# PRBonn/LiDiff

Measured on NVIDIA H100. Metric: denoising_steps_per_sec_180k_pts_T50, higher is better.
Workload: dtype fp16x3 split tensor-core MMA, fp32 accumulate (fp32 CUDA cores for the Cin=3 stem), fp64 DPM update

## Files before the change

lidiff_b200/csrc/common.cuh:

```cuda
#pragma once
#include <cuda_runtime.h>
#include <stdint.h>
#include <stdio.h>
#include <string.h>
#include "../../include/lidiff_b200.h"

struct Lb2Handle {
    int      device;
    int      num_sms;
    int64_t  launches;
    int32_t* d_status;
    uint32_t configured;
    char     err[512];
};

enum { LB2_K_TC = 0, LB2_K_SCATTER = 4, LB2_K_NN_TABLE = 8, LB2_K_FPS_CLUSTER = 9, LB2_K_WGRAD = 10 };
template <class K>
static inline cudaError_t lb2_configure_smem(Lb2Handle* h, int bit, K kernel, int bytes) {
    if (h->configured & (1u << bit)) return cudaSuccess;
    cudaError_t e = cudaFuncSetAttribute(kernel, cudaFuncAttributeMaxDynamicSharedMemorySize, bytes);
    if (e == cudaSuccess) h->configured |= 1u << bit;
    return e;
}

static inline int lb2_fail(Lb2Handle* h, int code, const char* fmt, const char* a = "", const char* b = "") {
    if (h) snprintf(h->err, sizeof(h->err), fmt, a, b);
    return code;
}

#define LB2_POST_LAUNCH(h, name)                                                              \
    do {                                                                                      \
        (h)->launches++;                                                                      \
        cudaError_t e__ = cudaGetLastError();                                                 \
        if (e__ != cudaSuccess) return lb2_fail((h), LB2_ERR_CUDA, "%s: %s", name, cudaGetErrorString(e__)); \
    } while (0)

#define LB2_REQUIRE(h, cond, msg)                                                             \
    do { if (!(cond)) return lb2_fail((h), LB2_ERR_ARG, "bad argument: %s", msg); } while (0)

static inline unsigned cdiv(long long a, long long b) { return (unsigned)((a + b - 1) / b); }

size_t rs_sort_scratch_bytes(int n_cap, int nbits);
int rs_sort_keys(Lb2Handle* h, cudaStream_t s, const unsigned* keys, const int* d_n, int n_cap, int nbits, int* order, void* scratch);

#define LB2_AXIS_BITS 18
#define LB2_AXIS_OFF  (1 << (LB2_AXIS_BITS - 1))

__device__ __forceinline__ bool lb2_pack_key(int b, int x, int y, int z, unsigned long long& key) {
    unsigned ux = (unsigned)x + LB2_AXIS_OFF, uy = (unsigned)y + LB2_AXIS_OFF, uz = (unsigned)z + LB2_AXIS_OFF;
    const unsigned lim = 1u << LB2_AXIS_BITS;
    bool ok = ((unsigned)b < 1024u) && ux < lim && uy < lim && uz < lim;
    if (!ok) {
        b = min(max(b, 0), 1023);
        ux = min(ux, lim - 1); uy = min(uy, lim - 1); uz = min(uz, lim - 1);
        if (x < -LB2_AXIS_OFF) ux = 0;
        if (y < -LB2_AXIS_OFF) uy = 0;
        if (z < -LB2_AXIS_OFF) uz = 0;
    }
    key = ((unsigned long long)b << (3 * LB2_AXIS_BITS)) | ((unsigned long long)ux << (2 * LB2_AXIS_BITS))
        | ((unsigned long long)uy << LB2_AXIS_BITS) | (unsigned long long)uz;
    return ok;
}

__device__ __forceinline__ unsigned lb2_hash(unsigned long long k) {
    k ^= k >> 33; k *= 0xff51afd7ed558ccdULL; k ^= k >> 33; k *= 0xc4ceb9fe1a85ec53ULL; k ^= k >> 33;
    return (unsigned)k;
}

#define LB2_MAP_AXIS_OFF (1 << (LB2_MAP_AXIS_BITS - 1))

template <class T>
__device__ __forceinline__ bool lb2_map_cell_ok(T f) { return f >= -(T)LB2_MAP_AXIS_OFF && f < (T)LB2_MAP_AXIS_OFF; }

__device__ __forceinline__ unsigned long long lb2_map_key_push(unsigned long long key, int cell) {
    return (key << LB2_MAP_AXIS_BITS) | (unsigned long long)(unsigned)(cell + LB2_MAP_AXIS_OFF);
}

__device__ __forceinline__ unsigned lb2_key_insert(unsigned long long* keys, unsigned mask, unsigned long long key) {
    unsigned s = lb2_hash(key) & mask;
    while (true) {
        unsigned long long kk = keys[s];
        if (kk == LB2_KEY_EMPTY) {
            kk = atomicCAS(keys + s, (unsigned long long)LB2_KEY_EMPTY, key);
            if (kk == LB2_KEY_EMPTY) return s;
        }
        if (kk == key) return s;
        s = (s + 1) & mask;
    }
}

__device__ __forceinline__ int lb2_grid_lookup(const unsigned long long* __restrict__ keys,
                                               const int* __restrict__ rows, unsigned mask,
                                               unsigned long long key) {
    unsigned slot = lb2_hash(key) & mask;
    while (true) {
        unsigned long long kk = __ldg(keys + slot);
        if (kk == key) return __ldg(rows + slot);
        if (kk == LB2_KEY_EMPTY) return -1;
        slot = (slot + 1) & mask;
    }
}

__device__ __forceinline__ int floor_to_multiple(int v, int ts) {
    int q = v / ts;
    if ((v % ts != 0) && ((v < 0) != (ts < 0))) --q;
    return q * ts;
}
```

lidiff_b200/csrc/spconv_tc.cu:

```cuda
#include "common.cuh"
#include <algorithm>
#include <stdlib.h>
#include "tc_common.cuh"

namespace tc {

constexpr int THREADS = 384;
constexpr int NUM_PRODUCER = 128;
constexpr int NUM_CONSUMER_WARPS = 8;
constexpr int STEP_BUDGET = 64;
constexpr int MAX_KVOL = 27;
constexpr int MAX_STAGES = 4;
constexpr int EPI_BATCH = 4;

struct Params {
    int c1, c2, cout, kvol;
    const unsigned char* wpacked;
    const float* scale;
    const float* shift;
    int relu;
    const int* nbr;
    long long nbr_stride;
    const int* d_mout;
    int mout_cap;
    const int* row_perm;
    const unsigned* row_mask;
    const int* tile_order;
    int stages, nchunks, group;
    int npass, nsplit;
    lb2_conv_io io[2];
    uint32_t range_mask, prior_mask;
    const float* partial_in;
    float* partial_out;
};

constexpr int PRODUCER_REGS = 88;
constexpr int CONSUMER_REGS = 208;
static_assert(128 * PRODUCER_REGS + 256 * CONSUMER_REGS <= THREADS * 168, "register split exceeds the CTA's allocation");

struct TileInfo {
    int idx[MAX_KVOL * BM];
    int row[BM];
    uint32_t mask[4];
    uint32_t prior[4];
    int item;
    int pad[3];
};
constexpr int NUM_BARS = 3 * MAX_STAGES + 4;

template <int NC>
__global__ void __launch_bounds__(THREADS, 1) k_spconv_tc(const Params p) {
    extern __shared__ unsigned char smem_raw[];
    const int M = p.d_mout ? min(*p.d_mout, p.mout_cap) : p.mout_cap;
    const int warp = threadIdx.x >> 5, lane = threadIdx.x & 31;
    const int ctot = p.c1 + p.c2;
    const int S = p.stages;

    const uint32_t raw = smem_u32(smem_raw);
    const uint32_t base = (raw + 1023u) & ~1023u;
    unsigned char* gen = smem_raw + (base - raw);
    constexpr uint32_t b_tile = (uint32_t)NC * 128u;
    const uint32_t b_full = (uint32_t)p.cout * 128u;
    const uint32_t stage_bytes = 2u * A_TILE + 2u * b_tile;
    TileInfo* info = reinterpret_cast<TileInfo*>(gen + (size_t)S * stage_bytes);
    const uint32_t bar0 = smem_u32(info + 2);
    auto full_a = [&](int s) { return bar0 + 8u * s; };
    auto full_b = [&](int s) { return bar0 + 8u * (MAX_STAGES + s); };
    auto empty = [&](int s) { return bar0 + 8u * (2 * MAX_STAGES + s); };
    auto info_full = [&](int b) { return bar0 + 8u * (3 * MAX_STAGES + b); };
    auto info_empty = [&](int b) { return bar0 + 8u * (3 * MAX_STAGES + 2 + b); };

    if (threadIdx.x == 0) {
        for (int s = 0; s < S; ++s) { mbar_init(full_a(s), NUM_PRODUCER); mbar_init(full_b(s), 1); mbar_init(empty(s), NUM_CONSUMER_WARPS); }
        for (int b = 0; b < 2; ++b) { mbar_init(info_full(b), NUM_PRODUCER); mbar_init(info_empty(b), NUM_CONSUMER_WARPS); }
        asm volatile("fence.mbarrier_init.release.cluster;" ::: "memory");
    }
    __syncthreads();

    if (warpgroup_role() == 0) {
        setmaxnreg_dec<PRODUCER_REGS>();
        const int sub = threadIdx.x & 7;
        const int rbase = threadIdx.x >> 3;
        const int D = max(S - 2, 0);
        int it = 0, arrived = 0;
        auto tile_of = [&](int x) {
            const int slot_i = x / (p.nsplit * p.npass);
            return slot_i * BM >= p.mout_cap ? -1 : p.tile_order ? __ldg(p.tile_order + slot_i) : slot_i;
        };
        auto load_row = [&](int tile) {
            const int slot = tile * BM + threadIdx.x;
            return (tile >= 0 && slot < M) ? (p.row_perm ? __ldg(p.row_perm + slot) : slot) : -1;
        };
        auto load_indices = [&](int& row, int (&v)[MAX_KVOL]) {
            const uint32_t m = row < 0 ? 0u : (p.row_mask ? __ldg(p.row_mask + row) : ~0u);
            const uint32_t want = m & p.range_mask;
#pragma unroll
            for (int k = 0; k < MAX_KVOL; ++k) {
                v[k] = -1;
                if (k < p.kvol && (want >> k) & 1u) v[k] = p.nbr ? __ldg(p.nbr + (long long)k * p.nbr_stride + row) : row;
            }
            if (m & p.prior_mask) row |= 1 << 30;
        };
        int x = blockIdx.x, tile = tile_of(x), row = load_row(tile), v[MAX_KVOL];
        load_indices(row, v);
        for (int j = 0;; ++j) {
            TileInfo& ti = info[j & 1];
            mbar_wait(info_empty(j & 1), ((j >> 1) & 1) ^ 1);
            if (tile < 0 || tile * BM >= M) {
                if (threadIdx.x == 0) ti.item = -1;
                mbar_arrive(info_full(j & 1));
                break;
            }
            {
                ti.row[threadIdx.x] = row < 0 ? row : row & ~(1 << 30);
                uint32_t have = 0;
#pragma unroll
                for (int k = 0; k < MAX_KVOL; ++k) {
                    if (k < p.kvol) {
                        ti.idx[k * BM + threadIdx.x] = v[k];
                        if (v[k] >= 0) have |= 1u << k;
                    }
                }
                const uint32_t wmask = __reduce_or_sync(0xffffffffu, have);
                const uint32_t wprior = __ballot_sync(0xffffffffu, row >= 0 && (row >> 30));
                if (lane == 0) { ti.mask[warp] = wmask; ti.prior[warp] = wprior; }
                if (threadIdx.x == 0) ti.item = x;
            }
            mbar_arrive(info_full(j & 1));
            mbar_wait(info_full(j & 1), (j >> 1) & 1);
            const uint32_t kmask = ti.mask[0] | ti.mask[1] | ti.mask[2] | ti.mask[3];
            const int x_next = x + gridDim.x;
            const int tile_next = tile_of(x_next);
            const int n0 = (x % p.nsplit) * NC;
            const lb2_conv_io io = p.io[(x / p.nsplit) % p.npass];
            const bool use_h = (io.in1_h != nullptr) && (p.c2 == 0 || io.in2_h != nullptr);
            for (uint32_t km = kmask; km; km &= km - 1) {
                const int k = __ffs(km) - 1;
                const int* idxk = ti.idx + k * BM;
                int src[8];
#pragma unroll
                for (int r = 0; r < 8; ++r) src[r] = idxk[rbase + 16 * r];
                for (int c = 0; c < p.nchunks; ++c) {
                    const int s = it % S;
                    mbar_wait(empty(s), ((it / S) & 1) ^ 1);
                    unsigned char* a_hi = gen + (size_t)s * stage_bytes;
                    const uint32_t a_hi_u = base + (uint32_t)s * stage_bytes;
                    if (threadIdx.x == 0) {
                        const uint32_t dst = a_hi_u + 2u * A_TILE;
                        const unsigned char* wsrc = p.wpacked + PACK_HEADER + ((size_t)k * p.nchunks + c) * (2u * b_full) + (size_t)n0 * 128u;
                        mbar_expect_tx(full_b(s), 2u * b_tile);
                        bulk_g2s(dst, wsrc, b_tile, full_b(s));
                        bulk_g2s(dst + b_tile, wsrc + b_full, b_tile, full_b(s));
                    }
                    const int ch = c * KC + sub * 8;
                    if (ch < ctot) {
                        const bool first = ch < p.c1;
                        const int cw = first ? p.c1 : p.c2;
                        const int co = first ? ch : ch - p.c1;
                        if (use_h) produce_a_split(reinterpret_cast<const __half*>(first ? io.in1_h : io.in2_h), cw, co, src, a_hi_u, a_hi_u + A_TILE, rbase, sub);
                        else produce_a_f32(first ? io.in1 : io.in2, cw, co, src, a_hi, a_hi + A_TILE, rbase, sub);
                    }
                    cp_async_commit();
                    ++it;
                    if (it - arrived > D) {
                        cp_async_wait_dyn(D);
                        fence_proxy_async();
                        mbar_arrive(full_a(arrived % S));
                        ++arrived;
                    }
                }
            }
            const int s = it % S;
            mbar_wait(empty(s), ((it / S) & 1) ^ 1);
            if (threadIdx.x == 0) mbar_arrive(full_b(s));
            ++it;
            x = x_next;
            tile = tile_next;
            row = load_row(tile);
            cp_async_wait<0>();
            fence_proxy_async();
            for (; arrived < it; ++arrived) mbar_arrive(full_a(arrived % S));
            load_indices(row, v);
        }
    } else {
        setmaxnreg_inc<CONSUMER_REGS>();
        const int wg = (warp >> 2) - 1;
        const float out_scale = __ldg(reinterpret_cast<const float*>(p.wpacked) + 1);
        int it = 0;
        for (int j = 0;; ++j) {
            const TileInfo& ti = info[j & 1];
            mbar_wait(info_full(j & 1), (j >> 1) & 1);
            const int x = ti.item;
            if (x < 0) break;
            const int n_off = __popc(ti.mask[0] | ti.mask[1] | ti.mask[2] | ti.mask[3]);
            float acc[NC / 2], tot[NC / 2];
            if (p.partial_in) {
                const int r0 = wg * 64 + (warp & 3) * 16 + (lane >> 2);
                const float* src[2];
#pragma unroll
                for (int hh = 0; hh < 2; ++hh) {
                    const int rr = r0 + 8 * hh;
                    const bool pr = (ti.prior[rr >> 5] >> (rr & 31)) & 1u;
                    src[hh] = pr ? p.partial_in + ((long long)((x / p.nsplit) % p.npass) * p.mout_cap + ti.row[rr]) * p.cout + (x % p.nsplit) * NC
                                 : nullptr;
                }
#pragma unroll
                for (int i = 0; i < NC / 2; i += 2) {
                    const float* q = src[(i >> 1) & 1];
                    const float2 t = q ? __ldcg(reinterpret_cast<const float2*>(q + 8 * (i >> 2) + 2 * (lane & 3))) : make_float2(-0.f, -0.f);
                    tot[i] = t.x;
                    tot[i + 1] = t.y;
                }
            } else {
#pragma unroll
                for (int i = 0; i < NC / 2; ++i) tot[i] = -0.f;
            }
            const int n_it = n_off * p.nchunks;
            int c = 0, in_group = 0, off_idx = 0, prev_s = -1;
            for (int i = 0; i < n_it; ++i, ++it) {
                const int s = it % S;
                const uint32_t par = (it / S) & 1;
                mbar_wait(full_b(s), par);
                mbar_wait(full_a(s), par);
                const uint32_t a_hi = base + (uint32_t)s * stage_bytes + (uint32_t)wg * (A_TILE / 2), a_lo = a_hi + A_TILE;
                const uint32_t b_hi = base + (uint32_t)s * stage_bytes + 2u * A_TILE, b_lo = b_hi + b_tile;
                const int ksteps = min(KC, ctot - c * KC) >> 4;
                reg_fence(acc);
                wg_stage_mma<NC>(acc, a_hi, a_lo, b_hi, b_lo, ksteps, in_group == 0 && c == 0);
                reg_fence(acc);
                wgmma_wait<1>();
                if (prev_s >= 0 && lane == 0) mbar_arrive(empty(prev_s));
                prev_s = s;
                if (++c < p.nchunks) continue;
                c = 0;
                ++off_idx;
                if (++in_group == p.group || off_idx == n_off) {
                    wgmma_wait<0>();
                    reg_fence(acc);
                    if (lane == 0) mbar_arrive(empty(prev_s));
                    prev_s = -1;
#pragma unroll
                    for (int i = 0; i < NC / 2; ++i) tot[i] = __fadd_rn(tot[i], acc[i]);
                    in_group = 0;
                }
            }
            wgmma_wait<0>();
            const int se = it % S;
            mbar_wait(full_b(se), (it / S) & 1);
            mbar_wait(full_a(se), (it / S) & 1);
            ++it;
            float* stage_c = reinterpret_cast<float*>(gen + (size_t)se * stage_bytes);
            {
                const int r0 = wg * 64 + (warp & 3) * 16 + (lane >> 2);
                const float sc = p.partial_out ? 1.f : out_scale;
#pragma unroll
                for (int i = 0; i < NC / 2; i += 2) {
                    const int row = r0 + 8 * ((i >> 1) & 1), col = 8 * (i >> 2) + 2 * (lane & 3);
                    *reinterpret_cast<float2*>(stage_c + row * NC + (((col >> 2) ^ (row & 7)) << 2) + (col & 3)) =
                        make_float2(tot[i] * sc, tot[i + 1] * sc);
                }
            }
            asm volatile("bar.sync 1, 256;" ::: "memory");
            const lb2_conv_io io = p.io[(x / p.nsplit) % p.npass];
            const int n0 = (x % p.nsplit) * NC;
            const int cw = warp - 4;
            constexpr int nv = NC >> 2;
            constexpr int PER_LANE = (BM / NUM_CONSUMER_WARPS) * nv / 32;
            static_assert(PER_LANE % EPI_BATCH == 0, "a lane's elements come in whole batches");
            const bool has_res = io.residual || io.residual_h;
            const bool gated = io.out_gated || io.out_gated_h;
            const float4 zero4 = make_float4(0.f, 0.f, 0.f, 0.f);
            if (p.partial_out) {
                float* dst = p.partial_out + (long long)((x / p.nsplit) % p.npass) * p.mout_cap * p.cout;
                for (int e = lane; e < PER_LANE * 32; e += 32) {
                    const int rr = cw + NUM_CONSUMER_WARPS * (e / nv);
                    const int lcol = (e % nv) * 4;
                    const int orow = ti.row[rr];
                    if (orow >= 0)
                        __stcg(reinterpret_cast<float4*>(dst + (long long)orow * p.cout + n0 + lcol),
                               *reinterpret_cast<const float4*>(stage_c + rr * NC + (((lcol >> 2) ^ (rr & 7)) << 2)));
                }
            }
            for (int e0 = 0; !p.partial_out && e0 < PER_LANE; e0 += EPI_BATCH) {
                int orow[EPI_BATCH], col[EPI_BATCH];
                long long gi[EPI_BATCH];
                float4 a4[EPI_BATCH], pre4[EPI_BATCH], s4[EPI_BATCH], h4[EPI_BATCH], res4[EPI_BATCH], g4[EPI_BATCH];
#pragma unroll
                for (int b = 0; b < EPI_BATCH; ++b) {
                    const int e = lane + 32 * (e0 + b);
                    const int rr = cw + NUM_CONSUMER_WARPS * (e / nv);
                    const int lcol = (e % nv) * 4;
                    col[b] = n0 + lcol;
                    orow[b] = ti.row[rr];
                    const bool live = orow[b] >= 0;
                    const long long ro = (long long)orow[b] * p.cout;
                    a4[b] = *reinterpret_cast<const float4*>(stage_c + rr * NC + (((lcol >> 2) ^ (rr & 7)) << 2));
                    pre4[b] = (live && io.pre_add) ? __ldg(reinterpret_cast<const float4*>(io.pre_add + ro + col[b])) : zero4;
                    s4[b] = p.scale ? __ldg(reinterpret_cast<const float4*>(p.scale + col[b])) : zero4;
                    h4[b] = p.scale ? __ldg(reinterpret_cast<const float4*>(p.shift + col[b])) : zero4;
                    res4[b] = (live && has_res) ? load_residual4(io.residual, io.residual_h, orow[b], p.cout, col[b]) : zero4;
                    gi[b] = (live && gated && io.gate_table && io.gate_idx) ? __ldg(io.gate_idx + orow[b]) : 0;
                }
#pragma unroll
                for (int b = 0; b < EPI_BATCH; ++b)
                    g4[b] = (orow[b] >= 0 && gated && io.gate_table) ? __ldg(reinterpret_cast<const float4*>(io.gate_table + gi[b] * p.cout + col[b])) : zero4;
#pragma unroll
                for (int b = 0; b < EPI_BATCH; ++b) {
                    if (orow[b] < 0) continue;
                    const long long ro = (long long)orow[b] * p.cout;
                    float y[4] = {a4[b].x, a4[b].y, a4[b].z, a4[b].w};
                    if (io.pre_add) {
                        y[0] += pre4[b].x; y[1] += pre4[b].y; y[2] += pre4[b].z; y[3] += pre4[b].w;
                    }
                    if (p.scale) {
                        y[0] = fmaf(y[0], s4[b].x, h4[b].x); y[1] = fmaf(y[1], s4[b].y, h4[b].y);
                        y[2] = fmaf(y[2], s4[b].z, h4[b].z); y[3] = fmaf(y[3], s4[b].w, h4[b].w);
                    }
                    if (has_res) {
                        y[0] += res4[b].x; y[1] += res4[b].y; y[2] += res4[b].z; y[3] += res4[b].w;
                    }
                    if (p.relu) {
#pragma unroll
                        for (int q = 0; q < 4; ++q) y[q] = fmaxf(y[q], 0.f);
                    }
                    if (io.out) *reinterpret_cast<float4*>(io.out + ro + col[b]) = make_float4(y[0], y[1], y[2], y[3]);
                    if (io.out_h) store_split4(io.out_h, orow[b], p.cout, col[b], y);
                    if (gated) {
                        if (io.gate_table) {
                            y[0] *= g4[b].x; y[1] *= g4[b].y; y[2] *= g4[b].z; y[3] *= g4[b].w;
                        }
                        if (io.out_gated) *reinterpret_cast<float4*>(io.out_gated + ro + col[b]) = make_float4(y[0], y[1], y[2], y[3]);
                        if (io.out_gated_h) store_split4(io.out_gated_h, orow[b], p.cout, col[b], y);
                    }
                }
            }
            fence_proxy_async();
            __syncwarp();
            if (lane == 0) {
                mbar_arrive(empty(se));
                mbar_arrive(info_empty(j & 1));
            }
        }
    }
}

__global__ void k_pack_weights(const float* __restrict__ w, int kvol, int cin, int cout, int nchunks, unsigned char* __restrict__ out) {
    const long long total = (long long)kvol * nchunks * cout * KC;
    long long t = (long long)blockIdx.x * blockDim.x + threadIdx.x;
    const float scale = weight_scale(*reinterpret_cast<const unsigned*>(out));
    if (t == 0) reinterpret_cast<float*>(out)[1] = 1.0f / scale;
    if (t >= total) return;
    const int kk = (int)(t % KC);
    const int n = (int)((t / KC) % cout);
    const int c = (int)((t / ((long long)KC * cout)) % nchunks);
    const int k = (int)(t / ((long long)KC * cout * nchunks));
    const int ch = c * KC + kk;
    const float v = ch < cin ? w[((long long)k * cin + ch) * cout + n] * scale : 0.f;
    const __half hi = __float2half_rn(v);
    const __half lo = __float2half_rn(v - __half2float(hi));
    const size_t tile = (size_t)cout * 128;
    unsigned char* blob = out + PACK_HEADER + ((size_t)k * nchunks + c) * 2 * tile;
    const uint32_t off = sw128(n, kk >> 3) + (uint32_t)(kk & 7) * 2u;
    *reinterpret_cast<__half*>(blob + off) = hi;
    *reinterpret_cast<__half*>(blob + tile + off) = lo;
}

static bool shape_ok(int c1, int c2, int cout, int kvol) {
    const int ctot = c1 + c2;
    if (kvol < 1 || kvol > MAX_KVOL) return false;
    if (ctot % 16 != 0 || ctot < 16) return false;
    if (c2 > 0 && (c1 % 8 != 0 || c2 % 8 != 0)) return false;
    if (cout % 32 != 0 || cout < 32 || cout > 256) return false;
    if (cout > 128 && cout != 256) return false;
    return true;
}

static size_t smem_bytes(int nc, int stages) {
    return 1024 + (size_t)stages * (2 * A_TILE + 2 * (size_t)nc * 128) + 2 * sizeof(TileInfo) + NUM_BARS * sizeof(uint64_t);
}

template <int NC>
static int launch(Lb2Handle* h, cudaStream_t s, const Params& p, int stages) {
    const size_t smem = smem_bytes(NC, stages);
    cudaError_t e = lb2_configure_smem(h, LB2_K_TC + (NC / 32 - 1), k_spconv_tc<NC>, (int)(227 * 1024));
    if (e != cudaSuccess) return lb2_fail(h, LB2_ERR_CUDA, "k_spconv_tc smem attribute: %s", cudaGetErrorString(e));
    const unsigned grid = (unsigned)std::min<long long>(h->num_sms, (long long)cdiv(p.mout_cap, BM) * p.npass * p.nsplit);
    k_spconv_tc<NC><<<grid, THREADS, smem, s>>>(p);
    LB2_POST_LAUNCH(h, "k_spconv_tc");
    return LB2_OK;
}

}

bool lb2_spconv_tc_supported(const lb2_conv_desc* d) { return tc::shape_ok(d->c1, d->c2, d->cout, d->kvol); }

extern "C" size_t lb2_packed_weight_bytes(int32_t kvol, int32_t cin, int32_t cout) {
    if (!tc::shape_ok(cin, 0, cout, kvol)) return 0;
    const int nchunks = (cin + tc::KC - 1) / tc::KC;
    return tc::PACK_HEADER + (size_t)kvol * nchunks * 2 * (size_t)cout * 128;
}

extern "C" int lb2_pack_weights(void* handle, void* stream, const float* weight, int32_t kvol, int32_t cin, int32_t cout, void* packed) {
    Lb2Handle* h = (Lb2Handle*)handle;
    LB2_REQUIRE(h, h && weight && packed, "pack_weights null");
    if (!tc::shape_ok(cin, 0, cout, kvol)) return lb2_fail(h, LB2_ERR_UNSUP, "pack_weights: shape not supported by the tensor-core variant%s", "");
    const int nchunks = (cin + tc::KC - 1) / tc::KC;
    const long long total = (long long)kvol * nchunks * cout * tc::KC;
    const long long nw = (long long)kvol * cin * cout;
    if (cudaMemsetAsync(packed, 0, tc::PACK_HEADER, (cudaStream_t)stream) != cudaSuccess) return lb2_fail(h, LB2_ERR_CUDA, "pack_weights memset%s", "");
    tc::k_weight_absmax<<<(unsigned)std::min<long long>(cdiv(nw, 256), 1024), 256, 0, (cudaStream_t)stream>>>(weight, nw, (unsigned*)packed);
    LB2_POST_LAUNCH(h, "k_weight_absmax");
    tc::k_pack_weights<<<cdiv(total, 256), 256, 0, (cudaStream_t)stream>>>(weight, kvol, cin, cout, nchunks, (unsigned char*)packed);
    LB2_POST_LAUNCH(h, "k_pack_weights");
    return LB2_OK;
}

int lb2_spconv_tc_launch(Lb2Handle* h, cudaStream_t s, const lb2_conv_desc* d) {
    tc::Params p;
    p.c1 = d->c1; p.c2 = d->c2; p.cout = d->cout; p.kvol = d->kvol;
    p.wpacked = (const unsigned char*)d->weight_packed;
    p.scale = d->scale; p.shift = d->shift; p.relu = d->relu;
    p.nbr = d->nbr; p.nbr_stride = d->nbr_stride; p.d_mout = d->d_mout; p.mout_cap = d->mout_cap; p.row_perm = d->row_perm;
    p.tile_order = d->nbr ? d->tile_order128 : nullptr;
    p.row_mask = d->nbr ? (const unsigned*)d->row_mask : nullptr;
    p.nchunks = (d->c1 + d->c2 + tc::KC - 1) / tc::KC;
    const int nsplit = d->cout > 128 ? 2 : 1;
    const int nc = d->cout / nsplit;
    p.npass = d->npass > 1 ? 2 : 1;
    p.nsplit = nsplit;
    int stages = tc::MAX_STAGES;
    while (stages > 2 && tc::smem_bytes(nc, stages) > 227 * 1024) --stages;
    p.stages = stages;
    const int steps_per_offset = 3 * ((d->c1 + d->c2 + 15) / 16);
    p.group = std::max(1, tc::STEP_BUDGET / steps_per_offset);
    p.io[0] = d->io[0]; p.io[1] = d->io[d->npass > 1 ? 1 : 0];
    p.range_mask = ~0u; p.prior_mask = 0u; p.partial_in = nullptr; p.partial_out = nullptr;
    if (d->k1 > 0) {
        if (d->kvol != 27 || !d->nbr || !d->row_mask || d->k0 < 0 || d->k0 >= d->k1 || d->k1 > 27 || p.group != 1 ||
            (d->k0 > 0) != (d->partial_in != nullptr) || (d->k1 < 27) != (d->partial_out != nullptr))
            return lb2_fail(h, LB2_ERR_ARG, "offset range: needs kvol 27, a map with row masks, c1 + c2 >= 176, 0 <= k0 < k1 <= 27, "
                                            "partial_in iff k0 > 0 and partial_out iff k1 < 27%s", "");
        p.range_mask = ((1u << d->k1) - 1u) & ~((1u << d->k0) - 1u);
        p.prior_mask = (1u << d->k0) - 1u;
        p.partial_in = d->partial_in;
        p.partial_out = d->partial_out;
    }
    switch (nc) {
        case 32: return tc::launch<32>(h, s, p, stages);
        case 64: return tc::launch<64>(h, s, p, stages);
        case 96: return tc::launch<96>(h, s, p, stages);
        case 128: return tc::launch<128>(h, s, p, stages);
        default: return lb2_fail(h, LB2_ERR_UNSUP, "tensor-core variant: no kernel for %s output channels per CTA", nc == 80 ? "80" : nc == 112 ? "112" : "this many");
    }
}
```

lidiff_b200/csrc/tc_common.cuh:

```cuda
#pragma once
#include <cuda_fp16.h>
#include <stdint.h>

namespace tc {

constexpr int BM = 128;
constexpr int KC = 64;
constexpr int A_TILE = BM * KC * 2;
constexpr int PACK_HEADER = 256;

__device__ __forceinline__ uint32_t smem_u32(const void* p) { return (uint32_t)__cvta_generic_to_shared(p); }

__device__ __forceinline__ void mbar_init(uint32_t bar, uint32_t count) {
    asm volatile("mbarrier.init.shared::cta.b64 [%0], %1;" ::"r"(bar), "r"(count) : "memory");
}
__device__ __forceinline__ void mbar_arrive(uint32_t bar) {
    asm volatile("mbarrier.arrive.shared::cta.b64 _, [%0];" ::"r"(bar) : "memory");
}
__device__ __forceinline__ void mbar_expect_tx(uint32_t bar, uint32_t bytes) {
    asm volatile("mbarrier.arrive.expect_tx.shared::cta.b64 _, [%0], %1;" ::"r"(bar), "r"(bytes) : "memory");
}
__device__ __forceinline__ void mbar_wait(uint32_t bar, uint32_t parity) {
    uint32_t ok = 0;
    while (!ok) {
        asm volatile("{\n\t.reg .pred p;\n\tmbarrier.try_wait.parity.shared::cta.b64 p, [%1], %2, %3;\n\tselp.u32 %0, 1, 0, p;\n\t}"
                     : "=r"(ok) : "r"(bar), "r"(parity), "r"(0x989680u) : "memory");
    }
}
__device__ __forceinline__ void bulk_g2s(uint32_t dst, const void* src, uint32_t bytes, uint32_t bar) {
    asm volatile("cp.async.bulk.shared::cluster.global.mbarrier::complete_tx::bytes [%0], [%1], %2, [%3];"
                 ::"r"(dst), "l"(src), "r"(bytes), "r"(bar) : "memory");
}
__device__ __forceinline__ void fence_proxy_async() { asm volatile("fence.proxy.async.shared::cta;" ::: "memory"); }

__device__ __forceinline__ uint64_t make_desc(uint32_t saddr) {
    return (uint64_t)((saddr >> 4) & 0x3FFFu) | ((uint64_t)1 << 16) | ((uint64_t)(1024 >> 4) << 32) | ((uint64_t)1 << 62);
}
__device__ __forceinline__ void wgmma_fence() { asm volatile("wgmma.fence.sync.aligned;" ::: "memory"); }
__device__ __forceinline__ void wgmma_commit() { asm volatile("wgmma.commit_group.sync.aligned;" ::: "memory"); }
template <int N>
__device__ __forceinline__ void wgmma_wait() { asm volatile("wgmma.wait_group.sync.aligned %0;" ::"n"(N) : "memory"); }

__device__ __forceinline__ void wgmma_m64n32(float* d, uint64_t da, uint64_t db, uint32_t accumulate) {
    asm volatile("{\n\t.reg .pred p;\n\tsetp.ne.b32 p, %18, 0;\n\t"
                 "wgmma.mma_async.sync.aligned.m64n32k16.f32.f16.f16 {%0, %1, %2, %3, %4, %5, %6, %7, %8, %9, %10, %11, %12, %13, %14, %15}, %16, %17, p, 1, 1, 0, 0;\n\t}"
        : "+f"(d[0]), "+f"(d[1]), "+f"(d[2]), "+f"(d[3]), "+f"(d[4]), "+f"(d[5]), "+f"(d[6]), "+f"(d[7]),
          "+f"(d[8]), "+f"(d[9]), "+f"(d[10]), "+f"(d[11]), "+f"(d[12]), "+f"(d[13]), "+f"(d[14]), "+f"(d[15])
        : "l"(da), "l"(db), "r"(accumulate) : "memory");
}
__device__ __forceinline__ void wgmma_m64n64(float* d, uint64_t da, uint64_t db, uint32_t accumulate) {
    asm volatile("{\n\t.reg .pred p;\n\tsetp.ne.b32 p, %34, 0;\n\t"
                 "wgmma.mma_async.sync.aligned.m64n64k16.f32.f16.f16 {%0, %1, %2, %3, %4, %5, %6, %7, %8, %9, %10, %11, %12, %13, %14, %15, %16, %17, %18, %19, %20, %21, %22, %23, %24, %25, %26, %27, %28, %29, %30, %31}, %32, %33, p, 1, 1, 0, 0;\n\t}"
        : "+f"(d[0]), "+f"(d[1]), "+f"(d[2]), "+f"(d[3]), "+f"(d[4]), "+f"(d[5]), "+f"(d[6]), "+f"(d[7]),
          "+f"(d[8]), "+f"(d[9]), "+f"(d[10]), "+f"(d[11]), "+f"(d[12]), "+f"(d[13]), "+f"(d[14]), "+f"(d[15]),
          "+f"(d[16]), "+f"(d[17]), "+f"(d[18]), "+f"(d[19]), "+f"(d[20]), "+f"(d[21]), "+f"(d[22]), "+f"(d[23]),
          "+f"(d[24]), "+f"(d[25]), "+f"(d[26]), "+f"(d[27]), "+f"(d[28]), "+f"(d[29]), "+f"(d[30]), "+f"(d[31])
        : "l"(da), "l"(db), "r"(accumulate) : "memory");
}
__device__ __forceinline__ void wgmma_m64n96(float* d, uint64_t da, uint64_t db, uint32_t accumulate) {
    asm volatile("{\n\t.reg .pred p;\n\tsetp.ne.b32 p, %50, 0;\n\t"
                 "wgmma.mma_async.sync.aligned.m64n96k16.f32.f16.f16 {%0, %1, %2, %3, %4, %5, %6, %7, %8, %9, %10, %11, %12, %13, %14, %15, %16, %17, %18, %19, %20, %21, %22, %23, %24, %25, %26, %27, %28, %29, %30, %31, "
                 "%32, %33, %34, %35, %36, %37, %38, %39, %40, %41, %42, %43, %44, %45, %46, %47}, %48, %49, p, 1, 1, 0, 0;\n\t}"
        : "+f"(d[0]), "+f"(d[1]), "+f"(d[2]), "+f"(d[3]), "+f"(d[4]), "+f"(d[5]), "+f"(d[6]), "+f"(d[7]),
          "+f"(d[8]), "+f"(d[9]), "+f"(d[10]), "+f"(d[11]), "+f"(d[12]), "+f"(d[13]), "+f"(d[14]), "+f"(d[15]),
          "+f"(d[16]), "+f"(d[17]), "+f"(d[18]), "+f"(d[19]), "+f"(d[20]), "+f"(d[21]), "+f"(d[22]), "+f"(d[23]),
          "+f"(d[24]), "+f"(d[25]), "+f"(d[26]), "+f"(d[27]), "+f"(d[28]), "+f"(d[29]), "+f"(d[30]), "+f"(d[31]),
          "+f"(d[32]), "+f"(d[33]), "+f"(d[34]), "+f"(d[35]), "+f"(d[36]), "+f"(d[37]), "+f"(d[38]), "+f"(d[39]),
          "+f"(d[40]), "+f"(d[41]), "+f"(d[42]), "+f"(d[43]), "+f"(d[44]), "+f"(d[45]), "+f"(d[46]), "+f"(d[47])
        : "l"(da), "l"(db), "r"(accumulate) : "memory");
}
__device__ __forceinline__ void wgmma_m64n128(float* d, uint64_t da, uint64_t db, uint32_t accumulate) {
    asm volatile("{\n\t.reg .pred p;\n\tsetp.ne.b32 p, %66, 0;\n\t"
                 "wgmma.mma_async.sync.aligned.m64n128k16.f32.f16.f16 {%0, %1, %2, %3, %4, %5, %6, %7, %8, %9, %10, %11, %12, %13, %14, %15, %16, %17, %18, %19, %20, %21, %22, %23, %24, %25, %26, %27, %28, %29, %30, %31, "
                 "%32, %33, %34, %35, %36, %37, %38, %39, %40, %41, %42, %43, %44, %45, %46, %47, %48, %49, %50, %51, %52, %53, %54, %55, %56, %57, %58, %59, %60, %61, %62, %63}, %64, %65, p, 1, 1, 0, 0;\n\t}"
        : "+f"(d[0]), "+f"(d[1]), "+f"(d[2]), "+f"(d[3]), "+f"(d[4]), "+f"(d[5]), "+f"(d[6]), "+f"(d[7]),
          "+f"(d[8]), "+f"(d[9]), "+f"(d[10]), "+f"(d[11]), "+f"(d[12]), "+f"(d[13]), "+f"(d[14]), "+f"(d[15]),
          "+f"(d[16]), "+f"(d[17]), "+f"(d[18]), "+f"(d[19]), "+f"(d[20]), "+f"(d[21]), "+f"(d[22]), "+f"(d[23]),
          "+f"(d[24]), "+f"(d[25]), "+f"(d[26]), "+f"(d[27]), "+f"(d[28]), "+f"(d[29]), "+f"(d[30]), "+f"(d[31]),
          "+f"(d[32]), "+f"(d[33]), "+f"(d[34]), "+f"(d[35]), "+f"(d[36]), "+f"(d[37]), "+f"(d[38]), "+f"(d[39]),
          "+f"(d[40]), "+f"(d[41]), "+f"(d[42]), "+f"(d[43]), "+f"(d[44]), "+f"(d[45]), "+f"(d[46]), "+f"(d[47]),
          "+f"(d[48]), "+f"(d[49]), "+f"(d[50]), "+f"(d[51]), "+f"(d[52]), "+f"(d[53]), "+f"(d[54]), "+f"(d[55]),
          "+f"(d[56]), "+f"(d[57]), "+f"(d[58]), "+f"(d[59]), "+f"(d[60]), "+f"(d[61]), "+f"(d[62]), "+f"(d[63])
        : "l"(da), "l"(db), "r"(accumulate) : "memory");
}

template <int N>
__device__ __forceinline__ void wgmma_n(float (&d)[N / 2], uint64_t da, uint64_t db, uint32_t accumulate) {
    static_assert(N == 32 || N == 64 || N == 96 || N == 128, "wgmma_n: N must be 32, 64, 96 or 128");
    if constexpr (N == 128) wgmma_m64n128(d, da, db, accumulate);
    else if constexpr (N == 96) wgmma_m64n96(d, da, db, accumulate);
    else if constexpr (N == 64) wgmma_m64n64(d, da, db, accumulate);
    else wgmma_m64n32(d, da, db, accumulate);
}
template <int N, int KSTEPS>
__device__ __forceinline__ void wg_stage_mma_k(float (&d)[N / 2], uint32_t a_hi, uint32_t a_lo, uint32_t b_hi, uint32_t b_lo, uint32_t acc0) {
    wgmma_fence();
#pragma unroll
    for (int ks = 0; ks < KSTEPS; ++ks) {
        const uint64_t dah = make_desc(a_hi + ks * 32), dal = make_desc(a_lo + ks * 32);
        const uint64_t dbh = make_desc(b_hi + ks * 32), dbl = make_desc(b_lo + ks * 32);
        wgmma_n<N>(d, dah, dbh, ks == 0 ? acc0 : 1u);
        wgmma_n<N>(d, dal, dbh, 1u);
        wgmma_n<N>(d, dah, dbl, 1u);
    }
    wgmma_commit();
}
template <int N>
__device__ __forceinline__ void wg_stage_mma(float (&d)[N / 2], uint32_t a_hi, uint32_t a_lo, uint32_t b_hi, uint32_t b_lo, int ksteps, bool first) {
    const uint32_t acc0 = first ? 0u : 1u;
    if (ksteps == 4) wg_stage_mma_k<N, 4>(d, a_hi, a_lo, b_hi, b_lo, acc0);
    else if (ksteps == 2) wg_stage_mma_k<N, 2>(d, a_hi, a_lo, b_hi, b_lo, acc0);
    else if (ksteps == 1) wg_stage_mma_k<N, 1>(d, a_hi, a_lo, b_hi, b_lo, acc0);
    else wg_stage_mma_k<N, 3>(d, a_hi, a_lo, b_hi, b_lo, acc0);
}
__device__ __forceinline__ int warpgroup_role() { return __shfl_sync(0xffffffffu, (int)(threadIdx.x >> 7), 0); }
template <int R>
__device__ __forceinline__ void setmaxnreg_dec() { asm volatile("setmaxnreg.dec.sync.aligned.u32 %0;" ::"n"(R)); }
template <int R>
__device__ __forceinline__ void setmaxnreg_inc() { asm volatile("setmaxnreg.inc.sync.aligned.u32 %0;" ::"n"(R)); }
template <int R>
__device__ __forceinline__ void reg_fence(float (&d)[R]) {
#pragma unroll
    for (int i = 0; i < R; ++i) asm volatile("" : "+f"(d[i])::"memory");
}

__device__ __forceinline__ uint32_t sw128(int row, int chunk) {
    return (uint32_t)((row >> 3) * 1024 + (row & 7) * 128 + ((chunk ^ (row & 7)) << 4));
}

__device__ __forceinline__ uint32_t cvt_f16x2_sat(float x, float y) {
    uint32_t d;
    asm("cvt.rn.satfinite.f16x2.f32 %0, %1, %2;" : "=r"(d) : "f"(y), "f"(x));
    return d;
}
__device__ __forceinline__ uint32_t cvt_f16x2_rn(float x, float y) {
    uint32_t d;
    asm("cvt.rn.f16x2.f32 %0, %1, %2;" : "=r"(d) : "f"(y), "f"(x));
    return d;
}
__device__ __forceinline__ void split2(float x0, float x1, uint32_t& hi, uint32_t& lo) {
    hi = cvt_f16x2_sat(x0, x1);
    const float2 f = __half22float2(*reinterpret_cast<const __half2*>(&hi));
    lo = cvt_f16x2_rn(x0 - f.x, x1 - f.y);
}
__device__ __forceinline__ void split1(float x, __half& hi, __half& lo) {
    uint32_t h, l;
    split2(x, 0.f, h, l);
    hi = __ushort_as_half((unsigned short)(h & 0xFFFFu));
    lo = __ushort_as_half((unsigned short)(l & 0xFFFFu));
}
__device__ __forceinline__ void split8(const float4& a, const float4& b, uint4& hi, uint4& lo) {
    split2(a.x, a.y, hi.x, lo.x);
    split2(a.z, a.w, hi.y, lo.y);
    split2(b.x, b.y, hi.z, lo.z);
    split2(b.z, b.w, hi.w, lo.w);
}

__device__ __forceinline__ void store_split4(void* base, long long row, int c, int col, const float (&y)[4]) {
    __half* rp = reinterpret_cast<__half*>(base) + row * 2 * c;
    uint2 uh, ul;
    split2(y[0], y[1], uh.x, ul.x);
    split2(y[2], y[3], uh.y, ul.y);
    *reinterpret_cast<uint2*>(rp + col) = uh;
    *reinterpret_cast<uint2*>(rp + c + col) = ul;
}
__device__ __forceinline__ float4 load_residual4(const float* res, const void* res_h, long long row, int c, int col) {
    if (res) return __ldg(reinterpret_cast<const float4*>(res + row * c + col));
    if (!res_h) return make_float4(0.f, 0.f, 0.f, 0.f);
    const __half* rp = reinterpret_cast<const __half*>(res_h) + row * 2 * c + col;
    const uint2 uh = __ldg(reinterpret_cast<const uint2*>(rp)), ul = __ldg(reinterpret_cast<const uint2*>(rp + c));
    const float2 h0 = __half22float2(*reinterpret_cast<const __half2*>(&uh.x)), h1 = __half22float2(*reinterpret_cast<const __half2*>(&uh.y));
    const float2 l0 = __half22float2(*reinterpret_cast<const __half2*>(&ul.x)), l1 = __half22float2(*reinterpret_cast<const __half2*>(&ul.y));
    return make_float4(h0.x + l0.x, h0.y + l0.y, h1.x + l1.x, h1.y + l1.y);
}

static __global__ void k_weight_absmax(const float* __restrict__ w, long long n, unsigned* __restrict__ header) {
    long long t = (long long)blockIdx.x * blockDim.x + threadIdx.x;
    float m = 0.f;
    for (; t < n; t += (long long)gridDim.x * blockDim.x) {
        const float a = fabsf(w[t]);
        if (isfinite(a)) m = fmaxf(m, a);
    }
#pragma unroll
    for (int o = 16; o > 0; o >>= 1) m = fmaxf(m, __shfl_xor_sync(0xffffffffu, m, o));
    if ((threadIdx.x & 31) == 0) atomicMax(header, __float_as_uint(m));
}

__device__ __forceinline__ float weight_scale(unsigned max_bits) {
    const float m = __uint_as_float(max_bits);
    if (!(m > 0.f) || !isfinite(m)) return 1.f;
    int e;
    frexpf(m, &e);
    return ldexpf(1.f, min(14 - e, 126));
}

__device__ __forceinline__ void cp_async16(uint32_t dst, const void* src, uint32_t src_bytes) {
    asm volatile("cp.async.cg.shared.global [%0], [%1], 16, %2;" ::"r"(dst), "l"(src), "r"(src_bytes) : "memory");
}
__device__ __forceinline__ void cp_async_commit() { asm volatile("cp.async.commit_group;" ::: "memory"); }
template <int N>
__device__ __forceinline__ void cp_async_wait() { asm volatile("cp.async.wait_group %0;" ::"n"(N) : "memory"); }
__device__ __forceinline__ void cp_async_wait_dyn(int n) {
    if (n <= 0) cp_async_wait<0>(); else if (n == 1) cp_async_wait<1>(); else if (n == 2) cp_async_wait<2>(); else cp_async_wait<3>();
}

__device__ __forceinline__ void produce_a_split(const __half* __restrict__ src_h, int cw, int co, const int (&src)[8],
                                                uint32_t a_hi, uint32_t a_lo, int rbase, int sub) {
#pragma unroll
    for (int j = 0; j < 8; ++j) {
        const uint32_t off = sw128(rbase + 16 * j, sub);
        const bool ok = src[j] >= 0;
        const __half* rp = src_h + (ok ? ((long long)src[j] * 2 * cw + co) : 0);
        cp_async16(a_hi + off, rp, ok ? 16u : 0u);
        cp_async16(a_lo + off, rp + (ok ? cw : 0), ok ? 16u : 0u);
    }
}
__device__ __forceinline__ void produce_a_f32(const float* __restrict__ srcp, int cw, int co, const int (&src)[8],
                                              unsigned char* a_hi, unsigned char* a_lo, int rbase, int sub) {
    float4 va[8], vb[8];
#pragma unroll
    for (int j = 0; j < 8; ++j) {
        if (src[j] >= 0) {
            const float4* rp = reinterpret_cast<const float4*>(srcp + (long long)src[j] * cw + co);
            va[j] = __ldg(rp);
            vb[j] = __ldg(rp + 1);
        } else {
            va[j] = make_float4(0.f, 0.f, 0.f, 0.f);
            vb[j] = va[j];
        }
    }
#pragma unroll
    for (int j = 0; j < 8; ++j) {
        uint4 hi, lo;
        split8(va[j], vb[j], hi, lo);
        const uint32_t off = sw128(rbase + 16 * j, sub);
        *reinterpret_cast<uint4*>(a_hi + off) = hi;
        *reinterpret_cast<uint4*>(a_lo + off) = lo;
    }
}

}
```

Before: 30.90.

## Run two CTAs per SM for the 32-channel tensor-core sparse conv kernel

Adds a second kernel instantiation with launch bounds of two CTAs per SM, used for output tiles of 32 channels. It shrinks the producer and consumer register budgets, halves the epilogue batch and the fp32 gather batch to fit, and sizes the smem ring so two CTAs share an SM. The grid doubles to 2x SMs. The aim is to hide gather and barrier latency on the narrow layers through extra occupancy, at the cost of fewer registers, possible spills and a shallower pipeline.

Result: no change. 31.13 (median of 6 runs) (+0.8%).

```diff
diff --git a/lidiff_b200/csrc/common.cuh b/lidiff_b200/csrc/common.cuh
--- a/lidiff_b200/csrc/common.cuh
+++ b/lidiff_b200/csrc/common.cuh
@@ -14,7 +14,7 @@
     char     err[512];
 };
 
-enum { LB2_K_TC = 0, LB2_K_SCATTER = 4, LB2_K_NN_TABLE = 8, LB2_K_FPS_CLUSTER = 9, LB2_K_WGRAD = 10 };
+enum { LB2_K_TC = 0, LB2_K_SCATTER = 4, LB2_K_NN_TABLE = 8, LB2_K_FPS_CLUSTER = 9, LB2_K_WGRAD = 10, LB2_K_TC2 = 12 };
 template <class K>
 static inline cudaError_t lb2_configure_smem(Lb2Handle* h, int bit, K kernel, int bytes) {
     if (h->configured & (1u << bit)) return cudaSuccess;
diff --git a/lidiff_b200/csrc/spconv_tc.cu b/lidiff_b200/csrc/spconv_tc.cu
--- a/lidiff_b200/csrc/spconv_tc.cu
+++ b/lidiff_b200/csrc/spconv_tc.cu
@@ -11,7 +11,7 @@
 constexpr int STEP_BUDGET = 64;
 constexpr int MAX_KVOL = 27;
 constexpr int MAX_STAGES = 4;
-constexpr int EPI_BATCH = 4;
+template <int CPS> constexpr int EPI_BATCH = CPS == 1 ? 4 : 2;
 
 struct Params {
     int c1, c2, cout, kvol;
@@ -34,9 +34,12 @@
     float* partial_out;
 };
 
-constexpr int PRODUCER_REGS = 88;
-constexpr int CONSUMER_REGS = 208;
-static_assert(128 * PRODUCER_REGS + 256 * CONSUMER_REGS <= THREADS * 168, "register split exceeds the CTA's allocation");
+constexpr int launch_regs(int cps) { return (65536 / (THREADS * cps)) & ~7; }
+template <int CPS> constexpr int PRODUCER_REGS = CPS == 1 ? 88 : 64;
+template <int CPS> constexpr int CONSUMER_REGS = CPS == 1 ? 208 : 88;
+template <int CPS> constexpr int F32_ROWS = CPS == 1 ? 8 : 4;
+static_assert(128 * PRODUCER_REGS<1> + 256 * CONSUMER_REGS<1> <= THREADS * launch_regs(1), "register split exceeds the CTA's allocation");
+static_assert(128 * PRODUCER_REGS<2> + 256 * CONSUMER_REGS<2> <= THREADS * launch_regs(2), "register split exceeds the CTA's allocation");
 
 struct TileInfo {
     int idx[MAX_KVOL * BM];
@@ -47,9 +50,16 @@
     int pad[3];
 };
 constexpr int NUM_BARS = 3 * MAX_STAGES + 4;
-
-template <int NC>
-__global__ void __launch_bounds__(THREADS, 1) k_spconv_tc(const Params p) {
+constexpr size_t smem_bytes(int nc, int stages) {
+    return 1024 + (size_t)stages * (2 * A_TILE + 2 * (size_t)nc * 128) + 2 * sizeof(TileInfo) + NUM_BARS * sizeof(uint64_t);
+}
+constexpr size_t SMEM_PER_SM = 228 * 1024, SMEM_RESERVED_PER_CTA = 1024;
+constexpr size_t smem_limit(int cps) { return SMEM_PER_SM / cps - SMEM_RESERVED_PER_CTA; }
+static_assert(smem_bytes(32, 2) <= smem_limit(2), "two CTAs of NC = 32 do not fit on an SM");
+static_assert(smem_bytes(64, 2) > smem_limit(2), "two CTAs of NC = 64 fit on an SM");
+
+template <int NC, int CPS>
+__device__ __forceinline__ void spconv_tc_body(const Params& p) {
     extern __shared__ unsigned char smem_raw[];
     const int M = p.d_mout ? min(*p.d_mout, p.mout_cap) : p.mout_cap;
     const int warp = threadIdx.x >> 5, lane = threadIdx.x & 31;
@@ -78,7 +88,7 @@
     __syncthreads();
 
     if (warpgroup_role() == 0) {
-        setmaxnreg_dec<PRODUCER_REGS>();
+        setmaxnreg_dec<PRODUCER_REGS<CPS>>();
         const int sub = threadIdx.x & 7;
         const int rbase = threadIdx.x >> 3;
         const int D = max(S - 2, 0);
@@ -158,7 +168,7 @@
                         const int cw = first ? p.c1 : p.c2;
                         const int co = first ? ch : ch - p.c1;
                         if (use_h) produce_a_split(reinterpret_cast<const __half*>(first ? io.in1_h : io.in2_h), cw, co, src, a_hi_u, a_hi_u + A_TILE, rbase, sub);
-                        else produce_a_f32(first ? io.in1 : io.in2, cw, co, src, a_hi, a_hi + A_TILE, rbase, sub);
+                        else produce_a_f32<F32_ROWS<CPS>>(first ? io.in1 : io.in2, cw, co, src, a_hi, a_hi + A_TILE, rbase, sub);
                     }
                     cp_async_commit();
                     ++it;
@@ -183,7 +193,7 @@
             load_indices(row, v);
         }
     } else {
-        setmaxnreg_inc<CONSUMER_REGS>();
+        setmaxnreg_inc<CONSUMER_REGS<CPS>>();
         const int wg = (warp >> 2) - 1;
         const float out_scale = __ldg(reinterpret_cast<const float*>(p.wpacked) + 1);
         int it = 0;
@@ -266,7 +276,7 @@
             const int cw = warp - 4;
             constexpr int nv = NC >> 2;
             constexpr int PER_LANE = (BM / NUM_CONSUMER_WARPS) * nv / 32;
-            static_assert(PER_LANE % EPI_BATCH == 0, "a lane's elements come in whole batches");
+            static_assert(PER_LANE % EPI_BATCH<CPS> == 0, "a lane's elements come in whole batches");
             const bool has_res = io.residual || io.residual_h;
             const bool gated = io.out_gated || io.out_gated_h;
             const float4 zero4 = make_float4(0.f, 0.f, 0.f, 0.f);
@@ -281,12 +291,12 @@
                                *reinterpret_cast<const float4*>(stage_c + rr * NC + (((lcol >> 2) ^ (rr & 7)) << 2)));
                 }
             }
-            for (int e0 = 0; !p.partial_out && e0 < PER_LANE; e0 += EPI_BATCH) {
-                int orow[EPI_BATCH], col[EPI_BATCH];
-                long long gi[EPI_BATCH];
-                float4 a4[EPI_BATCH], pre4[EPI_BATCH], s4[EPI_BATCH], h4[EPI_BATCH], res4[EPI_BATCH], g4[EPI_BATCH];
-#pragma unroll
-                for (int b = 0; b < EPI_BATCH; ++b) {
+            for (int e0 = 0; !p.partial_out && e0 < PER_LANE; e0 += EPI_BATCH<CPS>) {
+                int orow[EPI_BATCH<CPS>], col[EPI_BATCH<CPS>];
+                long long gi[EPI_BATCH<CPS>];
+                float4 a4[EPI_BATCH<CPS>], pre4[EPI_BATCH<CPS>], s4[EPI_BATCH<CPS>], h4[EPI_BATCH<CPS>], res4[EPI_BATCH<CPS>], g4[EPI_BATCH<CPS>];
+#pragma unroll
+                for (int b = 0; b < EPI_BATCH<CPS>; ++b) {
                     const int e = lane + 32 * (e0 + b);
                     const int rr = cw + NUM_CONSUMER_WARPS * (e / nv);
                     const int lcol = (e % nv) * 4;
@@ -302,10 +312,10 @@
                     gi[b] = (live && gated && io.gate_table && io.gate_idx) ? __ldg(io.gate_idx + orow[b]) : 0;
                 }
 #pragma unroll
-                for (int b = 0; b < EPI_BATCH; ++b)
+                for (int b = 0; b < EPI_BATCH<CPS>; ++b)
                     g4[b] = (orow[b] >= 0 && gated && io.gate_table) ? __ldg(reinterpret_cast<const float4*>(io.gate_table + gi[b] * p.cout + col[b])) : zero4;
 #pragma unroll
-                for (int b = 0; b < EPI_BATCH; ++b) {
+                for (int b = 0; b < EPI_BATCH<CPS>; ++b) {
                     if (orow[b] < 0) continue;
                     const long long ro = (long long)orow[b] * p.cout;
                     float y[4] = {a4[b].x, a4[b].y, a4[b].z, a4[b].w};
@@ -343,6 +353,11 @@
         }
     }
 }
+
+template <int NC>
+__global__ void __launch_bounds__(THREADS, 1) k_spconv_tc(const Params p) { spconv_tc_body<NC, 1>(p); }
+template <int NC>
+__global__ void __launch_bounds__(THREADS, 2) k_spconv_tc2(const Params p) { spconv_tc_body<NC, 2>(p); }
 
 __global__ void k_pack_weights(const float* __restrict__ w, int kvol, int cin, int cout, int nchunks, unsigned char* __restrict__ out) {
     const long long total = (long long)kvol * nchunks * cout * KC;
@@ -375,18 +390,30 @@
     return true;
 }
 
-static size_t smem_bytes(int nc, int stages) {
-    return 1024 + (size_t)stages * (2 * A_TILE + 2 * (size_t)nc * 128) + 2 * sizeof(TileInfo) + NUM_BARS * sizeof(uint64_t);
-}
-
-template <int NC>
-static int launch(Lb2Handle* h, cudaStream_t s, const Params& p, int stages) {
-    const size_t smem = smem_bytes(NC, stages);
-    cudaError_t e = lb2_configure_smem(h, LB2_K_TC + (NC / 32 - 1), k_spconv_tc<NC>, (int)(227 * 1024));
+static int ctas_per_sm(int nc) {
+    if (nc != 32) return 1;
+    const char* env = getenv("LB2_TC_CPS");
+    return env && env[0] == '1' && env[1] == '\0' ? 1 : 2;
+}
+
+static int ring_stages(int nc, int cps) {
+    int stages = MAX_STAGES;
+    while (stages > 2 && smem_bytes(nc, stages) > smem_limit(cps)) --stages;
+    return stages;
+}
+
+template <int NC, int CPS>
+static int launch(Lb2Handle* h, cudaStream_t s, Params p) {
+    p.stages = ring_stages(NC, CPS);
+    const size_t smem = smem_bytes(NC, p.stages);
+    void (*kernel)(const Params);
+    if constexpr (CPS == 1) kernel = k_spconv_tc<NC>;
+    else kernel = k_spconv_tc2<NC>;
+    cudaError_t e = lb2_configure_smem(h, (CPS == 1 ? LB2_K_TC : LB2_K_TC2) + (NC / 32 - 1), kernel, (int)smem_limit(CPS));
     if (e != cudaSuccess) return lb2_fail(h, LB2_ERR_CUDA, "k_spconv_tc smem attribute: %s", cudaGetErrorString(e));
-    const unsigned grid = (unsigned)std::min<long long>(h->num_sms, (long long)cdiv(p.mout_cap, BM) * p.npass * p.nsplit);
-    k_spconv_tc<NC><<<grid, THREADS, smem, s>>>(p);
-    LB2_POST_LAUNCH(h, "k_spconv_tc");
+    const unsigned grid = (unsigned)std::min<long long>((long long)CPS * h->num_sms, (long long)cdiv(p.mout_cap, BM) * p.npass * p.nsplit);
+    kernel<<<grid, THREADS, smem, s>>>(p);
+    LB2_POST_LAUNCH(h, CPS == 1 ? "k_spconv_tc" : "k_spconv_tc2");
     return LB2_OK;
 }
 
@@ -428,9 +455,6 @@
     const int nc = d->cout / nsplit;
     p.npass = d->npass > 1 ? 2 : 1;
     p.nsplit = nsplit;
-    int stages = tc::MAX_STAGES;
-    while (stages > 2 && tc::smem_bytes(nc, stages) > 227 * 1024) --stages;
-    p.stages = stages;
     const int steps_per_offset = 3 * ((d->c1 + d->c2 + 15) / 16);
     p.group = std::max(1, tc::STEP_BUDGET / steps_per_offset);
     p.io[0] = d->io[0]; p.io[1] = d->io[d->npass > 1 ? 1 : 0];
@@ -446,10 +470,10 @@
         p.partial_out = d->partial_out;
     }
     switch (nc) {
-        case 32: return tc::launch<32>(h, s, p, stages);
-        case 64: return tc::launch<64>(h, s, p, stages);
-        case 96: return tc::launch<96>(h, s, p, stages);
-        case 128: return tc::launch<128>(h, s, p, stages);
+        case 32: return tc::ctas_per_sm(32) == 2 ? tc::launch<32, 2>(h, s, p) : tc::launch<32, 1>(h, s, p);
+        case 64: return tc::launch<64, 1>(h, s, p);
+        case 96: return tc::launch<96, 1>(h, s, p);
+        case 128: return tc::launch<128, 1>(h, s, p);
         default: return lb2_fail(h, LB2_ERR_UNSUP, "tensor-core variant: no kernel for %s output channels per CTA", nc == 80 ? "80" : nc == 112 ? "112" : "this many");
     }
 }
diff --git a/lidiff_b200/csrc/tc_common.cuh b/lidiff_b200/csrc/tc_common.cuh
--- a/lidiff_b200/csrc/tc_common.cuh
+++ b/lidiff_b200/csrc/tc_common.cuh
@@ -215,28 +215,33 @@
         cp_async16(a_lo + off, rp + (ok ? cw : 0), ok ? 16u : 0u);
     }
 }
+template <int ROWS = 8>
 __device__ __forceinline__ void produce_a_f32(const float* __restrict__ srcp, int cw, int co, const int (&src)[8],
                                               unsigned char* a_hi, unsigned char* a_lo, int rbase, int sub) {
-    float4 va[8], vb[8];
-#pragma unroll
-    for (int j = 0; j < 8; ++j) {
-        if (src[j] >= 0) {
-            const float4* rp = reinterpret_cast<const float4*>(srcp + (long long)src[j] * cw + co);
-            va[j] = __ldg(rp);
-            vb[j] = __ldg(rp + 1);
-        } else {
-            va[j] = make_float4(0.f, 0.f, 0.f, 0.f);
-            vb[j] = va[j];
+    static_assert(8 % ROWS == 0, "whole batches of rows");
+#pragma unroll
+    for (int j0 = 0; j0 < 8; j0 += ROWS) {
+        float4 va[ROWS], vb[ROWS];
+#pragma unroll
+        for (int j = 0; j < ROWS; ++j) {
+            if (src[j0 + j] >= 0) {
+                const float4* rp = reinterpret_cast<const float4*>(srcp + (long long)src[j0 + j] * cw + co);
+                va[j] = __ldg(rp);
+                vb[j] = __ldg(rp + 1);
+            } else {
+                va[j] = make_float4(0.f, 0.f, 0.f, 0.f);
+                vb[j] = va[j];
+            }
         }
-    }
-#pragma unroll
-    for (int j = 0; j < 8; ++j) {
-        uint4 hi, lo;
-        split8(va[j], vb[j], hi, lo);
-        const uint32_t off = sw128(rbase + 16 * j, sub);
-        *reinterpret_cast<uint4*>(a_hi + off) = hi;
-        *reinterpret_cast<uint4*>(a_lo + off) = lo;
-    }
-}
-
-}
+#pragma unroll
+        for (int j = 0; j < ROWS; ++j) {
+            uint4 hi, lo;
+            split8(va[j], vb[j], hi, lo);
+            const uint32_t off = sw128(rbase + 16 * (j0 + j), sub);
+            *reinterpret_cast<uint4*>(a_hi + off) = hi;
+            *reinterpret_cast<uint4*>(a_lo + off) = lo;
+        }
+    }
+}
+
+}
```
